# szpiech/garlic

Measured on AMD Instinct MI355X. Metric: LOD-windows/sec (SNPs x inds / winsize), higher is better.
Workload: dtype f64

## Files before the change

### garlic_amd/csrc/garlic_hip.hip

```cpp
#include "../../include/garlic_hip.h"
#include "lod_kernels.hpp"
#include "variant_kernels.hpp"
#include "ld_kernels.hpp"
#include "tgls_ring_kernel.hpp"
#include "wlod_strip_kernel.hpp"
#include "wlod_small_kernel.hpp"
#include "coverage_kernel.hpp"
#include "roh_segments_kernel.hpp"
#include "feed_kernel.hpp"
#include "wlod_feed_kernel.hpp"

#include <algorithm>
#include <chrono>
#include <functional>
#include <mutex>
#include <queue>
#include <cmath>
#include <cstdarg>
#include <cstdio>
#include <cstdlib>
#include <cstring>
#include <string>
#include <thread>
#include <tuple>
// ... 124 lines not shown
};

static int score_alloc(garlic_ctx *ctx, size_t bytes, void **out);
static int score_free(garlic_ctx *ctx, void *ptr);

template <class T> struct PoolBuf : NoCopy {
    T *p = nullptr;
    garlic_ctx *ctx = nullptr;
    ~PoolBuf() { release(); }
    int reserve(garlic_ctx *c, size_t n)
    {
        release();
        void *q = nullptr;
        const int rc = score_alloc(c, std::max<size_t>(n, 1) * sizeof(T), &q);
        if (rc) return rc;
        p = (T *)q;
        ctx = c;
        return GARLIC_OK;
    }
    void release()
    {
        if (p) (void)score_free(ctx, p);
        p = nullptr;
    }
};


struct garlic_panel {
    garlic_ctx *ctx = nullptr;
    int32_t nchr = 0;
    int32_t nind = 0;
    int64_t nloci = 0;
    int64_t nind_pad = 0;
    int64_t nwordrows = 0;
    std::vector<int32_t> chr_nloci;
    std::vector<int64_t> chr_off;
    std::vector<int32_t> pos, cs, ce;
    std::vector<double> gpos, freq;
    bool have_map = false, have_freq = false, have_geno = false, have_gpos = false;
    DevBuf<uint32_t> d_packed;
    DevBuf<int32_t> d_pos, d_cs, d_ce;
    DevBuf<int64_t> d_chr_off;
    DevBuf<double> d_tab;
    bool tab_valid = false;
    double tab_error = 0;
    double tab_min = 0, tabgl_min = 0, glterms_min = 0;
    bool tab_all_finite = false;
    bool seg_valid = false;
    int32_t seg_max_gap = 0;
    std::vector<int64_t> boundaries;
    DevBuf<int32_t> d_blk_counts, d_blk_offsets, d_total;
    DevBuf<int64_t> d_boundaries;
    DevBuf<ChainItem> d_items;
    DevBuf<FeedItem> d_feed_items;
    DevBuf<FillItem> d_fill;
    DevBuf<int32_t> d_counter;
    DevBuf<ChrDev> d_chrs;
    DevBuf<int16_t> d_stage16;
    DevBuf<int64_t> d_row_counts;
    bool have_gl = false;
    std::vector<double> gl_values;
    std::unordered_map<uint64_t, int> gl_code;
    DevBuf<uint8_t> d_codes;
    DevBuf<double> d_tabgl;
    bool tabgl_valid = false;
    DevBuf<double> d_glterms;
    bool glterms_valid = false, glterms_scaled = false;
    int32_t glterms_M = 0;
    double glterms_mu = 0.0;

    int tabgl_ncodes = 0;
    bool gl_cont = false;
    DevBuf<double> d_glval;
    bool gl_vals_dropped = false;
    bool gl_cover_required = false;
    std::vector<uint8_t> gl_cover;
    DevBuf<double> d_freq;
    bool dfreq_valid = false;
    int gl_terms_by = 0;
    bool have_ld = false, wlod_use_gl = false, rld_valid = false;
    int32_t last_chain_kind = 0;
    int32_t last_feed_form = GARLIC_FEED_FROM_SCORES;
    int64_t last_feed_doubles = 0;
    int32_t ld_winsize = 0;
    DevBuf<double> d_rld, d_decay, d_stage64;
    DevBuf<uint64_t> d_phase;
    uint64_t geno_epoch = 0;
    CovBits cov_pending{nullptr, nullptr, 0.0};
    bool cov_written = false;
    bool have_phase = false;
    struct {
        DevBuf<uint64_t> sub, m, h, o;
        DevBuf<int32_t> loc, pair, loc_planes;
        DevBuf<double> hf, fwd, bwd, ld;
        DevBuf<LdSumChr> sum_chrs;
        DevBuf<LdPairChr> pair_chrs;
        uint64_t planes_key = 0;
        bool planes_valid = false;
        bool fuse_request = false, fused_done = false;
        void release()
        {
            sub.release(); m.release(); h.release(); o.release(); loc.release(); pair.release(); loc_planes.release();
            hf.release(); fwd.release(); bwd.release(); ld.release(); sum_chrs.release(); pair_chrs.release();
            planes_valid = false;
        }
    } lds;
// ... 916 lines not shown
    if (wlod_shape_ok && use_gl && (rc = ensure_gl_terms(p, true, c.M, c.mu))) return rc;
    f.wlod_gl = wlod_shape_ok && use_gl && p->glterms_valid && p->glterms_scaled;
    f.wlod_tuned = (wlod_shape_ok && !use_gl) || f.wlod_gl;
    if (f.wlod_tuned && !f.wlod_gl && sizeof(double) * (size_t)(W + TILE) * 4 + 16 > 150 * 1024) f.wlod_tuned = false;
    if (f.wlod_tuned && !f.wlod_gl && (rc = ensure_score_rows(p, c.error, c.M, c.mu, W))) return rc;
    if (!f.wlod_tuned && (rc = ensure_rld(p))) return rc;
    const bool wlod_stream = f.wlod_tuned && wlod_small && !f.cov_bits && !getenv("GARLIC_WLOD_SMALL_TILES");
    if (f.cov_bits && !f.wlod_tuned) return GARLIC_INTERNAL_NO_BITS;
    if (wlod_stream && (rc = ensure_rld(p))) return rc;
    if (use_gl && p->gl_cont && !f.wlod_tuned && (rc = ensure_gl_terms(p))) return rc;
    if (!f.wlod_tuned) {
        f.family = Family::wlod_generic;
        return GARLIC_OK;
    }
    f.writes_bits = true;
    f.no_prefetch = getenv("GARLIC_WLOD_NO_PF") != nullptr;
    const size_t wlod_rows = f.wlod_gl ? 0 : sizeof(double) * (size_t)(W + TILE) * 4;
    const size_t wlod_patch = sizeof(double) * (size_t)WAVE * WT_PITCH;
    const bool wlod_use_patch = wlod_rows + 16 + wlod_patch <= 160 * 1024 / 8 && !getenv("GARLIC_WLOD_NO_PATCH");
    const bool wlod_gl_ring = f.wlod_gl && !wlod_small && (c.ind_begin & (WAVE - 1)) == 0 && !getenv("GARLIC_WLOD_GL_NO_RING");
    const bool ring_patch = !getenv("GARLIC_WLOD_GL_NO_PATCH");
    const int strip_waves = (W + 15 - 16 * WS_WAVES <= 16 || getenv("GARLIC_WLOD_STRIP_NARROW_ONLY")) ? WS_WAVES : WS_WAVES_WIDE;
    const bool wlod_gl_strip = wlod_gl_ring && W + 15 - 16 * strip_waves <= 16 && !getenv("GARLIC_WLOD_GL_NO_STRIP");
    f.strip_waves = strip_waves;
    f.use_patch = wlod_gl_ring ? ring_patch : wlod_use_patch;
    f.tile_lds = wlod_gl_ring ? WLOD_GL_RING_OFF + (size_t)WLOD_WAVES * GARLIC_WLOD_GL_RING_ROWS * WAVE * 8
                              : wlod_rows + 16 + (wlod_use_patch ? wlod_patch : 0);
    f.strip_force_rerun = wlod_gl_strip && getenv("GARLIC_WLOD_STRIP_FORCE_RERUN") != nullptr;
    f.family = wlod_stream                            ? Family::wlod_stream
               : wlod_small                           ? Family::wlod_small_tiles
               : wlod_gl_strip                        ? Family::wlod_strip
               : wlod_gl_ring                         ? Family::wlod_glring
               : f.wlod_gl                            ? Family::wlod_tile_gl
               : !getenv("GARLIC_WLOD_ONE_BLOCK")     ? Family::wlod_tile2
                                                      : Family::wlod_tile;
    return GARLIC_OK;
}

void finish_form(const garlic_panel *p, const LodCall &c, const Layout &L, const double *d_out, LodForm &f)
{
    f.aligned16 = (c.pitch_align % 2 == 0) && ((reinterpret_cast<uintptr_t>(d_out) & 15) == 0);
    if (f.family == Family::wlod_stream && !f.aligned16) f.family = Family::wlod_small_tiles;
    f.strip_three = f.family == Family::wlod_strip && f.strip_waves != WS_WAVES_WIDE && f.aligned16 && !f.cov_bits &&
                    !getenv("GARLIC_WLOD_STRIP_TWO_PER_CU");
    for (int k = 0; f.strip_three && k < p->nchr; k++) f.strip_three = L.pitch[k] * 8 < ((int64_t)1 << 32);
}

using Plan = garlic_panel::Plan;

struct LodWork {
    std::vector<Run> runs;
    std::vector<FillItem> fill;
    std::vector<ChainItem> items;
    std::vector<FeedItem> feed_items;
    std::vector<ChrDev> chrs;
    std::vector<uint8_t> valid;
    std::vector<int2> tiles, segs;
    std::vector<WlodStrip> strips;
    std::vector<int32_t> feed_blocks;
};

int plan_lod(garlic_panel *p, const LodCall &c, const LodForm &form, const Layout &L, const garlic_panel::PlanKey &key, LodWork &w, Plan &plan)
{
    plan = Plan{false, key};
    const int nblk = (c.ind_count + WAVE - 1) / WAVE;
    int rc;
    p->plan.valid = false;
    plan_runs(p, c.W, w.runs, w.fill, plan.n_valid);
    const std::vector<int> order = longest_first(w.runs);
    w.items.reserve(w.runs.size() * nblk);
    for (size_t i = 0; i < order.size(); i++) {
        const Run &r = w.runs[order[i]];
        for (int k = 0; k < nblk; k++)
            if (!c.blocks || (*c.blocks)[(size_t)k]) w.items.push_back(ChainItem{r.chr, r.a, r.b, k * WAVE});
    }
    if (form.family == Family::feed) {
        std::vector<int32_t> col0(w.runs.size());
        for (size_t i = 0; i < w.runs.size(); i++) {
            const int32_t s = (w.runs[i].a + c.thin_step - 1) / c.thin_step;
            col0[i] = (int64_t)s * c.thin_step <= w.runs[i].b ? s : -1;
        }
        build_feed_items(w.runs, order, c.blocks, nblk, col0, w.feed_items);
        plan.n_feed_items = w.feed_items.size();
    }
    w.chrs.resize(p->nchr);
    for (int k = 0; k < p->nchr; k++)
        w.chrs[k] = ChrDev{p->chr_off[k], L.base[k], L.pitch[k], p->chr_nloci[k],
                           (c.pitch_align >= 2 && 64 * L.pitch[k] * 8 + 512 < ((int64_t)1 << 32)) ? 1 : 0};
    plan.n_items = w.items.size();
    plan.n_fill = w.fill.size();
    plan.n_runs = (int64_t)w.runs.size();
    if (!p->d_counter.p) {
        if ((rc = p->d_counter.reserve(8))) return rc;
        HIP_TRY(hipMemsetAsync(p->d_counter.p, 0, 8 * sizeof(int32_t), p->ctx->stream));
    }
    if (form.wlod_tuned || form.family == Family::wlod_feed) {
        w.valid.assign((size_t)p->nloci, 0);
        for (const Run &r : w.runs)
            memset(w.valid.data() + p->chr_off[r.chr] + r.a, 1, (size_t)(r.b - r.a + 1));
    }
    if (form.family == Family::wlod_feed) {
        for (int k = 0; k < p->nchr; k++) {
            const int32_t cols = (int32_t)(((int64_t)p->chr_nloci[k] + c.thin_step - 1) / c.thin_step);
            for (int32_t c0 = 0; c0 < cols; c0 += WFD_COLS) w.tiles.push_back(make_int2(k, c0));
        }
        plan.n_tiles = (int32_t)w.tiles.size();
        for (int k = 0; k < nblk; k++)
            if (!c.blocks || (*c.blocks)[(size_t)k]) w.feed_blocks.push_back(k);
        plan.n_feed_blocks = (int32_t)w.feed_blocks.size();
    }
    if (form.wlod_tuned) {
        for (int k = 0; k < p->nchr; k++)
            for (int s0 = 0; s0 < p->chr_nloci[k]; s0 += TILE) w.tiles.push_back(make_int2(k, s0));
        plan.n_tiles = (int32_t)w.tiles.size();
        for (int k = 0; k < p->nchr; k++)
            for (int s0 = 0; s0 < p->chr_nloci[k]; s0 += WSM_T) w.segs.push_back(make_int2(k, s0));
        plan.n_segs = (int32_t)w.segs.size();
    }
    if (form.family == Family::wlod_strip) {
        int64_t total_groups = 0;
        for (int k = 0; k < p->nchr; k++) total_groups += (p->chr_nloci[k] + WLOD_R - 1) / WLOD_R;
        const int64_t pairs = (nblk + 1) / 2;
        int64_t per = total_groups * pairs / 8192;
        per = std::min<int64_t>(256, std::max<int64_t>(64, per)) & ~(int64_t)1;
        if (const char *e = getenv("GARLIC_WLOD_STRIP_GROUPS")) per = std::max<int64_t>(1, atol(e));
        for (int k = 0; k < p->nchr; k++) {
            const int ng = (p->chr_nloci[k] + WLOD_R - 1) / WLOD_R;
            for (int g0 = 0; g0 < ng; g0 += (int)per)
                w.strips.push_back(WlodStrip{k, g0 * WLOD_R, std::min<int>((int)per, ng - g0), 0});
        }
        plan.n_strips = (int32_t)w.strips.size();
    }
    return GARLIC_OK;
}

int score_buffer(garlic_panel *p, const LodCall &c, const Layout &L, double **d_out)
{
    *d_out = c.out;
    if (c.where != GARLIC_HOST) return GARLIC_OK;
    int rc;
    if (p->d_out.cap < (size_t)L.total && c.mode == MODE_LOD && c.thin_step == 0 && !p->placing &&
// ... 75 lines not shown
int launch_wlod(garlic_panel *p, const LodCall &c, const LodForm &form, const Plan &plan, double *d_out)
{
    hipStream_t s = p->ctx->stream;
    const int nblk = (c.ind_count + WAVE - 1) / WAVE;
    const int per_wg = form.family == Family::wlod_tile2 ? WLOD2_BLOCKS : WLOD_WAVES;
    const int nquad = (nblk + per_wg - 1) / per_wg;
    const bool gl_ring = form.family == Family::wlod_glring || form.family == Family::wlod_strip;
    const int64_t score_rows = GOFF + p->nloci + GPAD_BACK;
    WlodArgs a{p->d_valid.p, p->d_chrs.p, p->d_tiles.p, p->nwordrows, p->nchr, c.ind_begin, c.ind_count, c.W, nquad,
               (uint32_t)((int64_t)plan.n_tiles * nquad), (form.use_patch ? 1 : 0) | (form.no_prefetch ? 2 : 0),
               score_rows, gl_ring ? 1 : 0, p->cov_pending, nullptr, nullptr};
    const uint32_t *a_packed = p->d_packed.p;
    const double *a_wtab = form.wlod_gl ? p->d_glterms.p : p->d_wtab.p, *a_skew = p->d_skew.p + SKEW_FRONT;
    const dim3 wl_block(WLOD_WAVES * WAVE);
    if (form.family == Family::wlod_stream) {
        a.tiles = p->d_segs.p;
        a.nquad = (nblk + WLOD2_BLOCKS - 1) / WLOD2_BLOCKS;
        a.n_work = (uint32_t)((int64_t)plan.n_segs * a.nquad);
        a.use_patch = 1;
        const void *fn = form.wlod_gl ? wlod_stream_small_gl_fn(c.W) : wlod_stream_small_fn(c.W);
        const size_t lds = wlod_small_lds_bytes(c.W);
        if (lds > 48 * 1024) HIP_TRY(hipFuncSetAttribute(fn, hipFuncAttributeMaxDynamicSharedMemorySize, (int)lds));
        const double *a_rld = p->d_rld.p;
        void *kargs[] = {(void *)&a_packed, (void *)&a_wtab, (void *)&a_rld, (void *)&d_out, (void *)&a};
        HIP_TRY(hipLaunchKernel(fn, dim3((a.n_work + 7u) / 8u * 8u), wl_block, kargs, lds, s));
        return GARLIC_OK;
    }
    if (form.family == Family::wlod_strip) {
        const int n_pairs = (nblk + 1) / 2;
        WlodStripArgs sa{p->d_valid.p, p->d_chrs.p, p->d_strips.p, p->d_glterms.p, a_skew, d_out,
                         score_rows, c.ind_begin, c.ind_count, c.W, form.strip_waves, n_pairs,
                         form.use_patch ? 1 : 0, (uint32_t)((int64_t)plan.n_strips * n_pairs), p->d_counter.p + 3, p->cov_pending};
        HIP_TRY(hipMemsetAsync(p->d_counter.p + 3, 0, sizeof(int32_t), s));
        const void *fn = form.strip_three ? (const void *)wlod_strip_gl3_kernel
                         : form.strip_waves == WS_WAVES_WIDE ? (form.aligned16 ? (const void *)wlod_strip_gl_kernel<true, WS_WAVES_WIDE>
                                                  : (const void *)wlod_strip_gl_kernel<false, WS_WAVES_WIDE>)
                                : (form.aligned16 ? (const void *)wlod_strip_gl_kernel<true, WS_WAVES>
                                                  : (const void *)wlod_strip_gl_kernel<false, WS_WAVES>);
        const uint32_t strip_lds = form.strip_three ? WF_LDS_BYTES : WS_LDS_BYTES;
        HIP_TRY(hipFuncSetAttribute(fn, hipFuncAttributeMaxDynamicSharedMemorySize, (int)strip_lds));
        void *kargs[] = {(void *)&sa};
        HIP_TRY(hipLaunchKernel(fn, dim3((sa.n_work + 7u) / 8u * 8u), dim3((form.strip_waves + 1) * WAVE), kargs, strip_lds, s));
        if (form.strip_force_rerun) HIP_TRY(hipMemsetAsync(p->d_counter.p + 3, 1, sizeof(int32_t), s));
        a.run_if = p->d_counter.p + 3;
        a.rerun_count = p->d_counter.p + 4;
    }
    const void *fn = wlod_tile_fn(form.family, form.wlod_gl, form.aligned16);
    if (form.tile_lds > 48 * 1024) HIP_TRY(hipFuncSetAttribute(fn, hipFuncAttributeMaxDynamicSharedMemorySize, (int)form.tile_lds));
    void *kargs[] = {(void *)&a_packed, (void *)&a_wtab, (void *)&a_skew, (void *)&d_out, (void *)&a};
    HIP_TRY(hipLaunchKernel(fn, dim3((a.n_work + 7u) / 8u * 8u), wl_block, kargs, form.tile_lds, s));
    return GARLIC_OK;
}

int launch_chain(garlic_panel *p, const LodCall &c, const LodForm &form, Plan &plan, const LodWork *fresh, int workers, double *d_out)
{
    garlic_ctx *ctx = p->ctx;
    ItemTrace trace;
    if (form.family == Family::feed && plan.n_feed_items) {
        FeedArgs f{p->d_packed.p, p->d_tab.p, p->d_feed_items.p, p->d_chrs.p, d_out, nullptr, p->nwordrows, c.ind_begin, c.ind_count, c.W,
                   (int32_t)plan.n_feed_items, c.thin_step, form.feed_asm ? 1 : 0, p->d_counter.p, nullptr};
        f.trace = trace.begin(8, plan.n_feed_items, "\n", ctx->stream);
        int grid = (int)std::min<size_t>(plan.n_feed_items, (size_t)ctx->n_cu * std::max(1, plan.feed_per_cu)), rc;
        if (fresh && (rc = feed_grid(ctx, fresh->feed_items, &grid, &plan.feed_per_cu))) return rc;
        void *kargs[] = {(void *)&f};
        HIP_TRY(hipLaunchKernel((const void *)lod_feed_kernel, dim3((unsigned)grid), dim3(FEED_G * WAVE), kargs, 0, ctx->stream));
    } else {
        ChainArgs a{p->d_packed.p, p->d_tab.p, p->d_items.p,     p->d_chrs.p,          d_out, p->nind_pad, p->nwordrows,
                    c.ind_begin,   c.ind_count, c.W,             (int32_t)plan.n_items, p->d_counter.p, nullptr};
        a.trace = trace.begin(4, plan.n_items, " 0\n", ctx->stream);
        if (form.aligned16)
            hipLaunchKernelGGL((lod_chain_kernel<true>), dim3((unsigned)workers), dim3(CHAIN_THREADS), 0, ctx->stream, a);
        else
            hipLaunchKernelGGL((lod_chain_kernel<false>), dim3((unsigned)workers), dim3(CHAIN_THREADS), 0, ctx->stream, a);
    }
    trace.write(ctx->stream);
    return GARLIC_OK;
}

int launch_tgls(garlic_panel *p, const LodCall &c, const LodForm &form, const Plan &plan, int workers, double *d_out)
{
    hipStream_t s = p->ctx->stream;
    const int64_t rows = GOFF + p->nloci + GPAD_BACK;
    if (form.cov_bits && !form.writes_bits) return GARLIC_INTERNAL_NO_BITS;
    if (form.family == Family::tgls_ring) {
        TglsArgs t{p->d_glterms.p, rows, p->d_items.p, p->d_chrs.p, d_out,
                   c.ind_begin, c.ind_count, c.W, (int32_t)plan.n_items, p->d_counter.p, p->cov_pending};
        if (form.cov_bits) p->cov_written = true;
        hipLaunchKernelGGL(lod_chain_ring_kernel, dim3((unsigned)workers), dim3(TG_THREADS), 0, s, t);
        return GARLIC_OK;
    }
    const VariantArgs a = variant_args(p, c, form, d_out);
    if (form.family == Family::tgls_terms)
        hipLaunchKernelGGL(lod_chain_terms_kernel, dim3((unsigned)plan.n_items), dim3(2 * WAVE), 0, s, a, (int)plan.n_items, rows, p->d_glterms.p);
    else
        hipLaunchKernelGGL(lod_chain_gl_kernel, dim3((unsigned)((plan.n_items + GL_WAVES - 1) / GL_WAVES)), dim3(GL_WAVES * WAVE), 0, s, a,
                           (int)plan.n_items);
    return GARLIC_OK;
}

int launch_generic_wlod(garlic_panel *p, const LodCall &c, const LodForm &form, const Plan &plan, double *d_out)
{
    const int ring = c.W + TILE;
    const size_t lds = sizeof(double) * ((size_t)ring * WAVE + ((c.W + 1) & ~1) + (size_t)WAVE * TPITCH);
    if (lds > 160 * 1024)
        return fail(GARLIC_ERR_INVALID, "wLOD with winsize %d: this build supports 2..240 and 16..4096", c.W);
    HIP_TRY(hipFuncSetAttribute(reinterpret_cast<const void *>(wlod_kernel), hipFuncAttributeMaxDynamicSharedMemorySize, (int)lds));
    hipLaunchKernelGGL(wlod_kernel, dim3((unsigned)plan.n_items), dim3(WAVE), lds, p->ctx->stream, variant_args(p, c, form, d_out), ring);
    return GARLIC_OK;
}

int launch_wlod_feed(garlic_panel *p, const LodCall &c, const LodForm &form, const Plan &plan, double *d_out)
{
    const int nquad = (plan.n_feed_blocks + WFD_WAVES - 1) / WFD_WAVES;
    WlodFeedArgs a{p->d_packed.p, form.wlod_gl ? p->d_glterms.p : p->d_wtab.p, p->d_skew.p + SKEW_FRONT, p->d_valid.p, p->d_chrs.p,
                   p->d_tiles.p, p->d_feed_blocks.p, d_out, p->nwordrows, GOFF + p->nloci + GPAD_BACK, c.ind_count, c.W, c.thin_step,
                   plan.n_feed_blocks, nquad, (uint32_t)((int64_t)plan.n_tiles * nquad)};
    if (!a.n_work) return GARLIC_OK;
    if (form.wlod_gl) hipLaunchKernelGGL(wlod_feed_kernel<true>, dim3(a.n_work), dim3(WFD_WAVES * WAVE), 0, p->ctx->stream, a);
    else hipLaunchKernelGGL(wlod_feed_kernel<false>, dim3(a.n_work), dim3(WFD_WAVES * WAVE), 0, p->ctx->stream, a);
    return GARLIC_OK;
}

int enqueue_lod(garlic_panel *p, const LodCall &c, const LodForm &form, const Layout &L, Plan &plan, const LodWork *fresh,
                double *d_out, Family family)
{
    garlic_ctx *ctx = p->ctx;
    hipStream_t s = ctx->stream;
    int rc = GARLIC_OK;
    HIP_TRY(hipEventRecord(ctx->ev_begin, s));
    if (fresh && ((rc = p->d_chrs.put(fresh->chrs, s)) || (rc = p->d_items.put(fresh->items, s)) || (rc = p->d_fill.put(fresh->fill, s)) ||
                  (rc = p->d_feed_items.put(fresh->feed_items, s)) || (rc = p->d_valid.put(fresh->valid, s)) ||
                  (rc = p->d_tiles.put(fresh->tiles, s)) || (rc = p->d_segs.put(fresh->segs, s)) || (rc = p->d_strips.put(fresh->strips, s)) ||
                  (rc = p->d_feed_blocks.put(fresh->feed_blocks, s))))
        return rc;
    if (family == Family::feed) {
        hipLaunchKernelGGL(fill_value_kernel, dim3(1024), dim3(256), 0, s, d_out, L.total, MISSING_D);
    } else if (plan.n_fill && !form.wlod_tuned && family != Family::wlod_feed && !form.cov_bits) {
        dim3 grid((unsigned)plan.n_fill, (unsigned)((c.ind_count + FILL_ROWS - 1) / FILL_ROWS));
        hipLaunchKernelGGL(fill_missing_kernel, grid, dim3(256), 0, s, p->d_fill.p, p->d_chrs.p, c.ind_count, d_out);
    }
    if (plan.n_items && (fresh || c.mode != MODE_LOD)) HIP_TRY(hipMemsetAsync(p->d_counter.p, 0, 2 * sizeof(int32_t), s));
    p->stats_slot = (int)(ctx->n_calls % garlic_ctx::HIST);
    HIP_TRY(hist_mark(ctx, false));
    int workers = ctx->n_cu;
    if (const char *e = getenv("GARLIC_WORKERS")) workers = std::max(1, atoi(e));
    workers = std::min<int>(workers, (int)plan.n_items);
    if (form.wlod_tuned || plan.n_items || family == Family::wlod_feed)
        switch (family) {
        case Family::chain:
        case Family::feed: rc = launch_chain(p, c, form, plan, fresh, workers, d_out); break;
        case Family::exact:
            hipLaunchKernelGGL(lod_chain_exact_kernel, dim3((unsigned)plan.n_items), dim3(WAVE), 0, s, variant_args(p, c, form, d_out),
                               (int)plan.n_items);
            break;
        case Family::tgls_ring:
        case Family::tgls_terms:
        case Family::tgls_lookup: rc = launch_tgls(p, c, form, plan, workers, d_out); break;
        case Family::wlod_generic: rc = launch_generic_wlod(p, c, form, plan, d_out); break;
        case Family::wlod_feed: rc = launch_wlod_feed(p, c, form, plan, d_out); break;
        default: rc = launch_wlod(p, c, form, plan, d_out);
        }
    if (rc) return rc;
    HIP_TRY(hist_mark(ctx, true));
    HIP_TRY(hipGetLastError());
    return GARLIC_OK;
}

int launch_lod(garlic_panel *p, Mode mode, int32_t W, double error, int32_t max_gap, int32_t M, double mu,
               int32_t ind_begin, int32_t ind_count, int32_t pitch_align, double *out, int32_t where,
               int32_t thin_step = 0, const std::vector<uint8_t> *blocks = nullptr)
{
    garlic_ctx *ctx = p->ctx;
    int rc;
    if ((rc = set_device(ctx))) return rc;
    const LodCall c{mode, W, max_gap, M, ind_begin, ind_count, where == GARLIC_HOST ? std::max(pitch_align, 32) : pitch_align,
                    thin_step, where, pitch_align, error, mu, out, blocks};
    LodForm form;
    if ((rc = check_lod_args(p, c)) || (rc = decide_form(p, c, form))) return rc;
    const Layout Lhost = make_layout(p, pitch_align, ind_count), L = make_layout(p, c.pitch_align, ind_count, thin_step);
    for (int k = 0; k < p->nchr; k++)
        if (3 * L.pitch[k] * 8 + 512 >= (int64_t)1 << 32)
            return fail(GARLIC_ERR_INVALID, "chromosome %d too long for 32-bit row offsets", k);
    double *d_out = nullptr;
    if ((rc = score_buffer(p, c, L, &d_out))) return rc;
    finish_form(p, c, L, d_out, form);

    garlic_panel::PlanKey key{(int)mode, W, max_gap, ind_begin, ind_count, c.pitch_align, thin_step, 0, form.wlod_tuned,
                form.family == Family::wlod_strip, thin_step > 0};
    if (blocks) {
// ... 1936 lines not shown
```

### garlic_amd/csrc/lod_kernels.hpp

```cpp
#pragma once
#include <hip/hip_runtime.h>
#include <stdint.h>

#include "chain_loop_gfx950.inc"

namespace garlic {

constexpr int WAVE = 64;
constexpr int TILE = 32;
constexpr int TPITCH = 34;
constexpr int GOFF = 32;
constexpr int GPAD_CHAIN = 32 * GARLIC_CHAIN_NSLOT + 48 * GARLIC_CHAIN_CHROWS + 64;
constexpr int GPAD_BACK = GPAD_CHAIN > 4160 ? GPAD_CHAIN : 4160;
constexpr double MISSING_D = -9999.0;

struct ChrDev {
    int64_t loc_base;
    int64_t out_base;
    int64_t out_pitch;
    int32_t nloci;
    int32_t fast;
};

struct ChainItem {
// ... 137 lines not shown
seg_scan_kernel(const int32_t *block_counts, int nblocks, int32_t *block_offsets, int32_t *total)
{
    int carry = 0;
    for (int base = 0; base < nblocks; base += WAVE) {
        int i = base + threadIdx.x;
        int v = (i < nblocks) ? block_counts[i] : 0;
        int inc = wave_inclusive_scan(v);
        if (i < nblocks) block_offsets[i] = carry + inc - v;
        carry += __shfl(inc, WAVE - 1, WAVE);
    }
    if (threadIdx.x == 0) *total = carry;
}

__global__ void __launch_bounds__(SEG_BLOCK)
seg_compact_kernel(const int32_t *pos, const int64_t *chr_off, const int32_t *cs,
                   const int32_t *ce, int nchr, int64_t nloci, int32_t max_gap,
                   const int32_t *block_offsets, int64_t *boundaries)
{
    __shared__ int wsum[SEG_BLOCK / WAVE];
    __shared__ int running;
    if (threadIdx.x == 0) running = block_offsets[blockIdx.x];
    int64_t base = (int64_t)blockIdx.x * SEG_BLOCK * SEG_ITEMS;
    __syncthreads();
    for (int k = 0; k < SEG_ITEMS; k++) {
        int64_t G = base + (int64_t)k * SEG_BLOCK + threadIdx.x;
        int f = boundary_flag(pos, chr_off, cs, ce, nchr, nloci, max_gap, G);
        int inc = wave_inclusive_scan(f);
        if ((threadIdx.x & 63) == 63) wsum[threadIdx.x >> 6] = inc;
        __syncthreads();
        int woff = 0;
        for (int w = 0; w < (int)(threadIdx.x >> 6); w++) woff += wsum[w];
        int start = running;
        if (f) boundaries[start + woff + inc - 1] = G;
        __syncthreads();
        if (threadIdx.x == SEG_BLOCK - 1) running = start + woff + inc;
        __syncthreads();
    }
}

constexpr int FILL_ROWS = 16;
__global__ void __launch_bounds__(256)
fill_missing_kernel(const FillItem *items, const ChrDev *chrs, int32_t nind, double *out)
{
    FillItem it = items[blockIdx.x];
    ChrDev c = chrs[it.chr];
    int wave = threadIdx.x >> 6, lane = threadIdx.x & 63;
    int row0 = blockIdx.y * FILL_ROWS;
    for (int r = row0 + wave; r < row0 + FILL_ROWS && r < nind; r += 4) {
        double *row = out + c.out_base + (int64_t)r * c.out_pitch;
        for (int l = it.lo + lane; l < it.hi; l += WAVE) row[l] = MISSING_D;
    }
}

struct ChainArgs {
    const uint32_t *packed;
    const double *tab;
    const ChainItem *items;
    const ChrDev *chrs;
    double *out;
    int64_t nind_pad;
    int64_t nwordrows;
    int32_t ind_begin;
    int32_t ind_count;
    int32_t winsize;
    int32_t n_items;
    int32_t *next_item;
    int64_t *trace;
};

constexpr uint32_t SLOT_BYTES = 3072;
constexpr uint32_t SL_LW1 = 0, SL_LW2 = 256, SL_TW1 = 512, SL_TW2 = 768;
constexpr uint32_t SL_LTAB = 1024, SL_TTAB = 2048;
constexpr uint32_t LDS_ITEM = 3072;
constexpr uint32_t LDS_TILE = GARLIC_CHAIN_LDS_TILE0;
constexpr uint32_t LDS_BYTES = GARLIC_CHAIN_LDS_TOTAL;
constexpr int CHAIN_THREADS = 256;

struct Streams {
    int64_t lead_w, trail_w;
    const double *lead_tab, *trail_tab;
    int sh_lead, sh_trail;
};

__device__ __forceinline__ void advance(Streams &st)
{
    st.lead_w += 2; st.trail_w += 2;
    st.lead_tab += 4 * TILE; st.trail_tab += 4 * TILE;
}

__device__ __forceinline__ void fill_regs(unsigned char *smem, const Streams &st,
                                          const uint32_t *gcol, int lane)
{
    const uint32_t l1 = gcol[(st.lead_w + 1) * WAVE], l2 = gcol[(st.lead_w + 2) * WAVE];
    const uint32_t t1 = gcol[(st.trail_w + 1) * WAVE], t2 = gcol[(st.trail_w + 2) * WAVE];
    const double2 tl = reinterpret_cast<const double2 *>(st.lead_tab)[lane];
    const double2 tt = reinterpret_cast<const double2 *>(st.trail_tab)[lane];
    *reinterpret_cast<uint32_t *>(smem + SL_LW1 + lane * 4) = l1;
    *reinterpret_cast<uint32_t *>(smem + SL_LW2 + lane * 4) = l2;
    *reinterpret_cast<uint32_t *>(smem + SL_TW1 + lane * 4) = t1;
    *reinterpret_cast<uint32_t *>(smem + SL_TW2 + lane * 4) = t2;
    *reinterpret_cast<double2 *>(smem + SL_LTAB + lane * 16) = tl;
    *reinterpret_cast<double2 *>(smem + SL_TTAB + lane * 16) = tt;
}

struct TileBits {
    uint32_t lead_lo, lead_hi, trail_lo, trail_hi;
};

template <int SLOT>
__device__ __forceinline__ TileBits tile_consume(const unsigned char *smem, uint32_t &lc,
                                                 uint32_t &tc, const Streams &st, int lane)
{
    const unsigned char *slot = smem + SLOT * SLOT_BYTES;
    const uint32_t l1 = *reinterpret_cast<const uint32_t *>(slot + SL_LW1 + lane * 4);
    const uint32_t l2 = *reinterpret_cast<const uint32_t *>(slot + SL_LW2 + lane * 4);
    const uint32_t t1 = *reinterpret_cast<const uint32_t *>(slot + SL_TW1 + lane * 4);
    const uint32_t t2 = *reinterpret_cast<const uint32_t *>(slot + SL_TW2 + lane * 4);
    TileBits tb;
    tb.lead_lo = __builtin_amdgcn_alignbit(l1, lc, st.sh_lead);
    tb.lead_hi = __builtin_amdgcn_alignbit(l2, l1, st.sh_lead);
    tb.trail_lo = __builtin_amdgcn_alignbit(t1, tc, st.sh_trail);
    tb.trail_hi = __builtin_amdgcn_alignbit(t2, t1, st.sh_trail);
    lc = l2;
    tc = t2;
    return tb;
}
// ... 6 lines not shown
    const unsigned char *slot = smem + SLOT * SLOT_BYTES;
    const uint32_t tile_lane = (uint32_t)lane * (TPITCH * 8);
#pragma unroll
    for (int j = 0; j < TILE; j++) {
        const uint32_t lw = (j < 16) ? tb.lead_lo : tb.lead_hi;
        const uint32_t tw = (j < 16) ? tb.trail_lo : tb.trail_hi;
        const uint32_t g1 = (lw >> (2 * (j & 15))) & 3u;
        const uint32_t g0 = (tw >> (2 * (j & 15))) & 3u;
        double t_in = *reinterpret_cast<const double *>(slot + SL_LTAB + j * 32 + g1 * 8);
        double t_out = *reinterpret_cast<const double *>(slot + SL_TTAB + j * 32 + g0 * 8);
        if (EDGE) {
            const int s = s0 + j;
            if (!(s > a && s <= b)) t_out = 0.0;
            if (!(s >= a && s <= b)) t_in = 0.0;
        }
        acc = (acc - t_out) + t_in;
        *reinterpret_cast<double *>(tile + tile_lane + j * 8) = acc;
    }
}

template <bool EDGE, bool ALIGNED16>
__device__ __forceinline__ void tile_store(const unsigned char *tile, int s0, int a, int b, int lane,
                                           int rows_valid, double *out_tile, int64_t pitch)
{
    const int rsub = lane >> 4, csub = lane & 15;
#pragma unroll
    for (int q = 0; q < WAVE / 4; q++) {
        const int qe = (4 * q < rows_valid) ? q : 0;
        const int re = min(rsub, rows_valid - 1 - 4 * qe);
        const double2 v = *reinterpret_cast<const double2 *>(
            tile + (uint32_t)(4 * qe + re) * (TPITCH * 8) + csub * 16);
        char *base = reinterpret_cast<char *>(out_tile + (int64_t)(4 * qe) * pitch);
        const uint32_t off = (uint32_t)re * (uint32_t)(pitch * 8) + (uint32_t)csub * 16u;
        double *dst = reinterpret_cast<double *>(base + off);
        if (EDGE) {
            const int s = s0 + 2 * csub;
            if (s >= a && s <= b) dst[0] = v.x;
            if (s + 1 >= a && s + 1 <= b) dst[1] = v.y;
        } else if (!ALIGNED16) {
            dst[0] = v.x;
            dst[1] = v.y;
        } else {
            *reinterpret_cast<double2 *>(dst) = v;
        }
    }
}

__global__ void __launch_bounds__(256) fill_value_kernel(double *dst, int64_t n, double value)
{
    for (int64_t i = (int64_t)blockIdx.x * blockDim.x + threadIdx.x; i < n; i += (int64_t)gridDim.x * blockDim.x)
        dst[i] = value;
}

template <bool ALIGNED16>
__global__ void __launch_bounds__(CHAIN_THREADS)
lod_chain_kernel(ChainArgs p)
{
    __shared__ __attribute__((aligned(16))) unsigned char smem[LDS_BYTES];
    unsigned char *tile = smem + LDS_TILE;
    const int lane = threadIdx.x & (WAVE - 1);
    const int wave = __builtin_amdgcn_readfirstlane(threadIdx.x >> 6);
    for (;;) {
    if (threadIdx.x == 0)
        *reinterpret_cast<int *>(smem + LDS_ITEM) = atomicAdd(p.next_item, 1);
    __syncthreads();
    const int item_idx =
        __builtin_amdgcn_readfirstlane(*reinterpret_cast<const int *>(smem + LDS_ITEM));
    __syncthreads();
    if (item_idx >= p.n_items) {
        if (threadIdx.x == 0) {
            __threadfence();
            if (atomicAdd(p.next_item + 1, 1) == (int)gridDim.x - 1) {
                p.next_item[0] = 0;
                p.next_item[1] = 0;
            }
        }
        return;
    }
    if (p.trace && threadIdx.x == 0) {
        p.trace[4 * item_idx + 0] = blockIdx.x;
        p.trace[4 * item_idx + 1] = wall_clock64();
    }
    const ChainItem it = p.items[item_idx];
    const ChrDev c = p.chrs[it.chr];
    const int W = p.winsize;
    const int a = it.a, b = it.b;
    const int rows_valid = min(WAVE, p.ind_count - it.ind0);
    const int64_t col0 = (int64_t)p.ind_begin + it.ind0;
    const uint32_t *gcol = p.packed + packed_index(0, col0 + lane, p.nwordrows);
    const int64_t Gbase = c.loc_base + GOFF;

    double acc = 0.0;
    if (wave == 0) {
        int l = a;
        const int lend = a + W - 1;
        while (l < lend) {
            const int64_t G = Gbase + l;
            const int sh = 2 * (int)(G & 15);
            const uint32_t *wp = gcol + (G >> 4) * WAVE;
            uint32_t wd[5];
#pragma unroll
            for (int q = 0; q < 5; q++) wd[q] = wp[q * WAVE];
            uint32_t al[4];
#pragma unroll
            for (int q = 0; q < 4; q++) al[q] = __builtin_amdgcn_alignbit(wd[q + 1], wd[q], sh);
            const int n = min(64, lend - l);
            double t[64];
#pragma unroll
            for (int q = 0; q < 64; q++) {
                const uint32_t g = (al[q >> 4] >> (2 * (q & 15))) & 3u;
                t[q] = p.tab[(G + min(q, n - 1)) * 4 + ((q < n) ? g : 3u)];
            }
#pragma unroll
            for (int q = 0; q < 64; q++) acc += (q < n) ? t[q] : 0.0;
            l += n;
        }
    }

    int s0 = a & ~(TILE - 1);
    Streams st;
    {
        const int64_t Glead = Gbase + s0 + W - 1;
        const int64_t Gtrail = Gbase + s0 - 1;
        st.sh_lead = 2 * (int)(Glead & 15);
        st.sh_trail = 2 * (int)(Gtrail & 15);
        st.lead_w = Glead >> 4;
        st.trail_w = Gtrail >> 4;
        st.lead_tab = p.tab + Glead * 4;
        st.trail_tab = p.tab + Gtrail * 4;
    }
    double *const out_row = p.out + c.out_base + (int64_t)it.ind0 * c.out_pitch;
    double *out_tile = out_row + s0;
    const int64_t pitch = c.out_pitch;

    for (int phase = 0; phase < 2; phase++) {
        const int last = (phase == 0) ? s0 : b;
        while (s0 <= last && s0 <= b) {
            if (wave == 0) {
                uint32_t lc = gcol[st.lead_w * WAVE];
                uint32_t tc = gcol[st.trail_w * WAVE];
                fill_regs(smem, st, gcol, lane);
                const TileBits tb = tile_consume<0>(smem, lc, tc, st, lane);
                tile_steps<true, 0>(smem, tile, acc, tb, s0, a, b, lane);
                tile_store<true, ALIGNED16>(tile, s0, a, b, lane, rows_valid, out_tile, pitch);
            }
            advance(st);
            s0 += TILE;
            out_tile += TILE;
        }
        if (phase == 1 || !ALIGNED16 || !c.fast || (col0 & 63) != 0) continue;
        if (st.lead_w - st.trail_w > GARLIC_CHAIN_MAX_DW) continue;

        int ntiles = (b + 1 - s0) / TILE;
        if (ntiles >= 2) {
            uint32_t lc = gcol[st.lead_w * WAVE];
            uint32_t tc = gcol[st.trail_w * WAVE];
            const int64_t chunk0 = st.trail_w / GARLIC_CHAIN_CHROWS;
            const int64_t chunkI = (st.lead_w + 2 * GARLIC_CHAIN_NSLOT) / GARLIC_CHAIN_CHROWS + 1;
            const uint32_t *pchunk =
                p.packed + packed_index(GARLIC_CHAIN_CHROWS * chunk0, col0, p.nwordrows);
            const uint32_t wmask = GARLIC_CHAIN_WROWS - 1;
            if (p.trace && threadIdx.x == 0) p.trace[4 * item_idx + 2] = wall_clock64();
            const uint32_t a_nchunk0 = (uint32_t)(chunkI - chunk0 + 1) * (GARLIC_CHAIN_CHROWS / 4);
            const uint32_t a_roff0 = (uint32_t)((GARLIC_CHAIN_CHROWS * chunk0) & wmask) * 256u;
            const uint32_t a_laddr0 = (uint32_t)(st.lead_w & wmask) * 256u;
            const uint32_t a_taddr0 = (uint32_t)(st.trail_w & wmask) * 256u;
            if (wave == 0) {
                uint32_t tin[4], tout[4];
#pragma unroll
                for (int q = 0; q < 4; q++) {
                    const uint32_t bb = 4u * (uint32_t)lane + (uint32_t)q;
                    const uint32_t sp = (bb & 3u) | (((bb >> 2) & 3u) << 8) | (((bb >> 4) & 3u) << 16) | (((bb >> 6) & 3u) << 24);
                    tin[q] = sp << 4;
                    tout[q] = sp << 6;
                }
                *reinterpret_cast<uint4 *>(smem + GARLIC_CHAIN_SPREAD_IN + lane * 16) = make_uint4(tin[0], tin[1], tin[2], tin[3]);
                *reinterpret_cast<uint4 *>(smem + GARLIC_CHAIN_SPREAD_OUT + lane * 16) = make_uint4(tout[0], tout[1], tout[2], tout[3]);
            }
            {
                asm volatile(GARLIC_CHAIN_LOOP_ASM
                             : [acc] "+v"(acc)
                             : [wave] "s"(wave), [lane] "v"(lane), [lc] "v"(lc), [tc] "v"(tc),
                               [pchunk] "s"(pchunk), [nchunk0] "s"(a_nchunk0), [roff0] "s"(a_roff0),
                               [laddr0] "s"(a_laddr0), [taddr0] "s"(a_taddr0),
                               [pltab] "s"(st.lead_tab), [pttab] "s"(st.trail_tab), [out] "s"(out_tile),
                               [ntiles] "s"(ntiles), [shl] "s"(st.sh_lead), [sht] "s"(st.sh_trail),
                               [pitch8] "s"((uint32_t)(pitch * 8)), [rows] "s"(rows_valid)
                             : GARLIC_CHAIN_LOOP_CLOBBERS);
            }
            st.lead_w += 2 * ntiles;
            st.trail_w += 2 * ntiles;
            st.lead_tab += (int64_t)(4 * TILE) * ntiles;
            st.trail_tab += (int64_t)(4 * TILE) * ntiles;
            s0 += ntiles * TILE;
            out_tile += (int64_t)ntiles * TILE;
            __syncthreads();
        }
    }
    if (p.trace && threadIdx.x == 0) p.trace[4 * item_idx + 3] = wall_clock64();
    }
}

}
```

Baseline: 7.293 billion.

## Split chain kernel into prep pass plus prefetched per-item start records

Moves each chain item's serial warm-up (initial window sum and first partial tile) into a separate chain_prep_kernel that runs one item per wave across many blocks, and also folds the missing-value fill into that launch. Per-item scalar setup (offsets, shifts, chunk addresses) is now computed on the host into 128-byte ChainStart records. The main persistent kernel has a spare wave fetch the next item index and record into LDS while the current item runs, so the atomic grab and setup latency overlap with work. The cost is an extra kernel launch, a device buffer for per-lane prep state, more host planning work, and a tail loop that now runs after the asm fast path rather than before it.

Measured after the change: 7.276 billion, median of 2. No clear change (-0.2%).

```diff
diff --git a/garlic_amd/csrc/garlic_hip.hip b/garlic_amd/csrc/garlic_hip.hip
--- a/garlic_amd/csrc/garlic_hip.hip
+++ b/garlic_amd/csrc/garlic_hip.hip
@@ -200,6 +200,8 @@
     DevBuf<int32_t> d_blk_counts, d_blk_offsets, d_total;
     DevBuf<int64_t> d_boundaries;
     DevBuf<ChainItem> d_items;
+    DevBuf<ChainStart> d_starts;
+    DevBuf<PrepRec> d_prep;
     DevBuf<FeedItem> d_feed_items;
     DevBuf<FillItem> d_fill;
     DevBuf<int32_t> d_counter;
@@ -1222,6 +1224,7 @@
     std::vector<Run> runs;
     std::vector<FillItem> fill;
     std::vector<ChainItem> items;
+    std::vector<ChainStart> starts;
     std::vector<FeedItem> feed_items;
     std::vector<ChrDev> chrs;
     std::vector<uint8_t> valid;
@@ -1229,6 +1232,46 @@
     std::vector<WlodStrip> strips;
     std::vector<int32_t> feed_blocks;
 };
+
+void chain_starts(const garlic_panel *p, const LodCall &c, const std::vector<ChrDev> &chrs, const std::vector<ChainItem> &items,
+                  std::vector<ChainStart> &starts)
+{
+    starts.resize(items.size());
+    for (size_t i = 0; i < items.size(); i++) {
+        const ChainItem &it = items[i];
+        const ChrDev &ch = chrs[(size_t)it.chr];
+        ChainStart &r = starts[i];
+        memset(&r, 0, sizeof(r));
+        const int64_t Gbase = ch.loc_base + GOFF;
+        const int64_t col0 = (int64_t)c.ind_begin + it.ind0;
+        r.a = it.a;
+        r.b = it.b;
+        r.s1 = (it.a & ~(TILE - 1)) + TILE;
+        r.rows_valid = std::min<int32_t>(WAVE, c.ind_count - it.ind0);
+        r.col0 = (int32_t)col0;
+        r.pitch = ch.out_pitch;
+        r.out_off = ch.out_base + (int64_t)it.ind0 * ch.out_pitch + r.s1;
+        const int64_t Glead = Gbase + r.s1 + c.W - 1, Gtrail = Gbase + r.s1 - 1;
+        r.sh_lead = 2 * (int32_t)(Glead & 15);
+        r.sh_trail = 2 * (int32_t)(Gtrail & 15);
+        r.lead_w = (int32_t)(Glead >> 4);
+        r.trail_w = (int32_t)(Gtrail >> 4);
+        r.lead_tab_off = Glead * 4;
+        r.trail_tab_off = Gtrail * 4;
+        const bool fast = ch.fast && (col0 & 63) == 0 && r.lead_w - r.trail_w <= GARLIC_CHAIN_MAX_DW;
+        const int32_t ntiles = r.s1 <= it.b ? (it.b + 1 - r.s1) / TILE : 0;
+        r.ntiles = (fast && ntiles >= 2) ? ntiles : 0;
+        const int64_t chunk0 = r.trail_w / GARLIC_CHAIN_CHROWS;
+        const int64_t chunkI = ((int64_t)r.lead_w + 2 * GARLIC_CHAIN_NSLOT) / GARLIC_CHAIN_CHROWS + 1;
+        const uint32_t wmask = GARLIC_CHAIN_WROWS - 1;
+        r.pchunk_off = packed_index(GARLIC_CHAIN_CHROWS * chunk0, col0, p->nwordrows);
+        r.nchunk0 = (uint32_t)(chunkI - chunk0 + 1) * (GARLIC_CHAIN_CHROWS / 4);
+        r.roff0 = (uint32_t)((GARLIC_CHAIN_CHROWS * chunk0) & wmask) * 256u;
+        r.laddr0 = (uint32_t)r.lead_w & wmask;
+        r.laddr0 *= 256u;
+        r.taddr0 = ((uint32_t)r.trail_w & wmask) * 256u;
+    }
+}
 
 int plan_lod(garlic_panel *p, const LodCall &c, const LodForm &form, const Layout &L, const garlic_panel::PlanKey &key, LodWork &w, Plan &plan)
 {
@@ -1257,6 +1300,7 @@
     for (int k = 0; k < p->nchr; k++)
         w.chrs[k] = ChrDev{p->chr_off[k], L.base[k], L.pitch[k], p->chr_nloci[k],
                            (c.pitch_align >= 2 && 64 * L.pitch[k] * 8 + 512 < ((int64_t)1 << 32)) ? 1 : 0};
+    if (c.mode == MODE_LOD && c.thin_step == 0) chain_starts(p, c, w.chrs, w.items, w.starts);
     plan.n_items = w.items.size();
     plan.n_fill = w.fill.size();
     plan.n_runs = (int64_t)w.runs.size();
@@ -1438,6 +1482,13 @@
     return GARLIC_OK;
 }
 
+ChainArgs chain_args(const garlic_panel *p, const LodCall &c, const Plan &plan, double *d_out)
+{
+    return ChainArgs{p->d_packed.p, p->d_tab.p, p->d_items.p, p->d_chrs.p, p->d_starts.p, p->d_prep.p, p->d_fill.p, d_out,
+                     p->nind_pad, p->nwordrows, c.ind_begin, c.ind_count, c.W, (int32_t)plan.n_items, (int32_t)plan.n_fill,
+                     p->d_counter.p, nullptr};
+}
+
 int launch_chain(garlic_panel *p, const LodCall &c, const LodForm &form, Plan &plan, const LodWork *fresh, int workers, double *d_out)
 {
     garlic_ctx *ctx = p->ctx;
@@ -1451,8 +1502,7 @@
         void *kargs[] = {(void *)&f};
         HIP_TRY(hipLaunchKernel((const void *)lod_feed_kernel, dim3((unsigned)grid), dim3(FEED_G * WAVE), kargs, 0, ctx->stream));
     } else {
-        ChainArgs a{p->d_packed.p, p->d_tab.p, p->d_items.p,     p->d_chrs.p,          d_out, p->nind_pad, p->nwordrows,
-                    c.ind_begin,   c.ind_count, c.W,             (int32_t)plan.n_items, p->d_counter.p, nullptr};
+        ChainArgs a = chain_args(p, c, plan, d_out);
         a.trace = trace.begin(4, plan.n_items, " 0\n", ctx->stream);
         if (form.aligned16)
             hipLaunchKernelGGL((lod_chain_kernel<true>), dim3((unsigned)workers), dim3(CHAIN_THREADS), 0, ctx->stream, a);
@@ -1515,12 +1565,17 @@
     int rc = GARLIC_OK;
     HIP_TRY(hipEventRecord(ctx->ev_begin, s));
     if (fresh && ((rc = p->d_chrs.put(fresh->chrs, s)) || (rc = p->d_items.put(fresh->items, s)) || (rc = p->d_fill.put(fresh->fill, s)) ||
+                  (rc = p->d_starts.put(fresh->starts, s)) || (rc = p->d_prep.reserve(fresh->starts.size() * WAVE)) ||
                   (rc = p->d_feed_items.put(fresh->feed_items, s)) || (rc = p->d_valid.put(fresh->valid, s)) ||
                   (rc = p->d_tiles.put(fresh->tiles, s)) || (rc = p->d_segs.put(fresh->segs, s)) || (rc = p->d_strips.put(fresh->strips, s)) ||
                   (rc = p->d_feed_blocks.put(fresh->feed_blocks, s))))
         return rc;
     if (family == Family::feed) {
         hipLaunchKernelGGL(fill_value_kernel, dim3(1024), dim3(256), 0, s, d_out, L.total, MISSING_D);
+    } else if (family == Family::chain) {
+        const ChainArgs a = chain_args(p, c, plan, d_out);
+        const size_t grid = (plan.n_items + 3) / 4 + plan.n_fill * (size_t)((c.ind_count + FILL_ROWS - 1) / FILL_ROWS);
+        if (grid) hipLaunchKernelGGL(chain_prep_kernel, dim3((unsigned)grid), dim3(256), 0, s, a);
     } else if (plan.n_fill && !form.wlod_tuned && family != Family::wlod_feed && !form.cov_bits) {
         dim3 grid((unsigned)plan.n_fill, (unsigned)((c.ind_count + FILL_ROWS - 1) / FILL_ROWS));
         hipLaunchKernelGGL(fill_missing_kernel, grid, dim3(256), 0, s, p->d_fill.p, p->d_chrs.p, c.ind_count, d_out);
diff --git a/garlic_amd/csrc/lod_kernels.hpp b/garlic_amd/csrc/lod_kernels.hpp
--- a/garlic_amd/csrc/lod_kernels.hpp
+++ b/garlic_amd/csrc/lod_kernels.hpp
@@ -213,11 +213,37 @@
     }
 }
 
+struct alignas(128) ChainStart {
+    int64_t out_off;
+    int64_t lead_tab_off;
+    int64_t trail_tab_off;
+    int64_t pchunk_off;
+    int64_t pitch;
+    int32_t a, b;
+    int32_t s1;
+    int32_t rows_valid;
+    int32_t ntiles;
+    int32_t col0;
+    int32_t lead_w, trail_w;
+    int32_t sh_lead, sh_trail;
+    uint32_t nchunk0, roff0, laddr0, taddr0;
+};
+constexpr int CHAIN_START_WORDS = 24;
+static_assert(sizeof(ChainStart) == 128 && offsetof(ChainStart, taddr0) == 4 * (CHAIN_START_WORDS - 1), "ChainStart layout");
+
+struct alignas(16) PrepRec {
+    double acc;
+    uint32_t lc, tc;
+};
+
 struct ChainArgs {
     const uint32_t *packed;
     const double *tab;
     const ChainItem *items;
     const ChrDev *chrs;
+    const ChainStart *starts;
+    PrepRec *prep;
+    const FillItem *fill;
     double *out;
     int64_t nind_pad;
     int64_t nwordrows;
@@ -225,6 +251,7 @@
     int32_t ind_count;
     int32_t winsize;
     int32_t n_items;
+    int32_t n_fill;
     int32_t *next_item;
     int64_t *trace;
 };
@@ -233,6 +260,7 @@
 constexpr uint32_t SL_LW1 = 0, SL_LW2 = 256, SL_TW1 = 512, SL_TW2 = 768;
 constexpr uint32_t SL_LTAB = 1024, SL_TTAB = 2048;
 constexpr uint32_t LDS_ITEM = 3072;
+constexpr uint32_t LDS_START = 3200;
 constexpr uint32_t LDS_TILE = GARLIC_CHAIN_LDS_TILE0;
 constexpr uint32_t LDS_BYTES = GARLIC_CHAIN_LDS_TOTAL;
 constexpr int CHAIN_THREADS = 256;
@@ -345,35 +373,31 @@
         dst[i] = value;
 }
 
-template <bool ALIGNED16>
-__global__ void __launch_bounds__(CHAIN_THREADS)
-lod_chain_kernel(ChainArgs p)
-{
-    __shared__ __attribute__((aligned(16))) unsigned char smem[LDS_BYTES];
-    unsigned char *tile = smem + LDS_TILE;
+constexpr uint32_t PREP_WAVE_LDS = SLOT_BYTES + WAVE * TPITCH * 8;
+__global__ void __launch_bounds__(256)
+chain_prep_kernel(ChainArgs p)
+{
+    __shared__ __attribute__((aligned(16))) unsigned char smem_all[4 * PREP_WAVE_LDS];
     const int lane = threadIdx.x & (WAVE - 1);
     const int wave = __builtin_amdgcn_readfirstlane(threadIdx.x >> 6);
-    for (;;) {
-    if (threadIdx.x == 0)
-        *reinterpret_cast<int *>(smem + LDS_ITEM) = atomicAdd(p.next_item, 1);
-    __syncthreads();
-    const int item_idx =
-        __builtin_amdgcn_readfirstlane(*reinterpret_cast<const int *>(smem + LDS_ITEM));
-    __syncthreads();
-    if (item_idx >= p.n_items) {
-        if (threadIdx.x == 0) {
-            __threadfence();
-            if (atomicAdd(p.next_item + 1, 1) == (int)gridDim.x - 1) {
-                p.next_item[0] = 0;
-                p.next_item[1] = 0;
-            }
+    const int n_head = (p.n_items + 3) >> 2;
+    if ((int)blockIdx.x >= n_head) {
+        const int row_groups = (p.ind_count + FILL_ROWS - 1) / FILL_ROWS;
+        const int f = ((int)blockIdx.x - n_head) / row_groups;
+        if (f >= p.n_fill) return;
+        const FillItem it = p.fill[f];
+        const ChrDev c = p.chrs[it.chr];
+        const int row0 = (((int)blockIdx.x - n_head) - f * row_groups) * FILL_ROWS;
+        for (int r = row0 + wave; r < row0 + FILL_ROWS && r < p.ind_count; r += 4) {
+            double *row = p.out + c.out_base + (int64_t)r * c.out_pitch;
+            for (int l = it.lo + lane; l < it.hi; l += WAVE) row[l] = MISSING_D;
         }
         return;
     }
-    if (p.trace && threadIdx.x == 0) {
-        p.trace[4 * item_idx + 0] = blockIdx.x;
-        p.trace[4 * item_idx + 1] = wall_clock64();
-    }
+    const int item_idx = (int)blockIdx.x * 4 + wave;
+    if (item_idx >= p.n_items) return;
+    unsigned char *smem = smem_all + wave * PREP_WAVE_LDS;
+    unsigned char *tile = smem + SLOT_BYTES;
     const ChainItem it = p.items[item_idx];
     const ChrDev c = p.chrs[it.chr];
     const int W = p.winsize;
@@ -384,33 +408,31 @@
     const int64_t Gbase = c.loc_base + GOFF;
 
     double acc = 0.0;
-    if (wave == 0) {
-        int l = a;
-        const int lend = a + W - 1;
-        while (l < lend) {
-            const int64_t G = Gbase + l;
-            const int sh = 2 * (int)(G & 15);
-            const uint32_t *wp = gcol + (G >> 4) * WAVE;
-            uint32_t wd[5];
-#pragma unroll
-            for (int q = 0; q < 5; q++) wd[q] = wp[q * WAVE];
-            uint32_t al[4];
-#pragma unroll
-            for (int q = 0; q < 4; q++) al[q] = __builtin_amdgcn_alignbit(wd[q + 1], wd[q], sh);
-            const int n = min(64, lend - l);
-            double t[64];
-#pragma unroll
-            for (int q = 0; q < 64; q++) {
-                const uint32_t g = (al[q >> 4] >> (2 * (q & 15))) & 3u;
-                t[q] = p.tab[(G + min(q, n - 1)) * 4 + ((q < n) ? g : 3u)];
-            }
-#pragma unroll
-            for (int q = 0; q < 64; q++) acc += (q < n) ? t[q] : 0.0;
-            l += n;
-        }
-    }
-
-    int s0 = a & ~(TILE - 1);
+    int l = a;
+    const int lend = a + W - 1;
+    while (l < lend) {
+        const int64_t G = Gbase + l;
+        const int sh = 2 * (int)(G & 15);
+        const uint32_t *wp = gcol + (G >> 4) * WAVE;
+        uint32_t wd[5];
+#pragma unroll
+        for (int q = 0; q < 5; q++) wd[q] = wp[q * WAVE];
+        uint32_t al[4];
+#pragma unroll
+        for (int q = 0; q < 4; q++) al[q] = __builtin_amdgcn_alignbit(wd[q + 1], wd[q], sh);
+        const int n = min(64, lend - l);
+        double t[64];
+#pragma unroll
+        for (int q = 0; q < 64; q++) {
+            const uint32_t g = (al[q >> 4] >> (2 * (q & 15))) & 3u;
+            t[q] = p.tab[(G + min(q, n - 1)) * 4 + ((q < n) ? g : 3u)];
+        }
+#pragma unroll
+        for (int q = 0; q < 64; q++) acc += (q < n) ? t[q] : 0.0;
+        l += n;
+    }
+
+    const int s0 = a & ~(TILE - 1);
     Streams st;
     {
         const int64_t Glead = Gbase + s0 + W - 1;
@@ -422,73 +444,131 @@
         st.lead_tab = p.tab + Glead * 4;
         st.trail_tab = p.tab + Gtrail * 4;
     }
-    double *const out_row = p.out + c.out_base + (int64_t)it.ind0 * c.out_pitch;
-    double *out_tile = out_row + s0;
-    const int64_t pitch = c.out_pitch;
-
-    for (int phase = 0; phase < 2; phase++) {
-        const int last = (phase == 0) ? s0 : b;
-        while (s0 <= last && s0 <= b) {
-            if (wave == 0) {
-                uint32_t lc = gcol[st.lead_w * WAVE];
-                uint32_t tc = gcol[st.trail_w * WAVE];
-                fill_regs(smem, st, gcol, lane);
-                const TileBits tb = tile_consume<0>(smem, lc, tc, st, lane);
-                tile_steps<true, 0>(smem, tile, acc, tb, s0, a, b, lane);
-                tile_store<true, ALIGNED16>(tile, s0, a, b, lane, rows_valid, out_tile, pitch);
+    double *out_tile = p.out + c.out_base + (int64_t)it.ind0 * c.out_pitch + s0;
+    uint32_t lc = gcol[st.lead_w * WAVE];
+    uint32_t tc = gcol[st.trail_w * WAVE];
+    fill_regs(smem, st, gcol, lane);
+    const TileBits tb = tile_consume<0>(smem, lc, tc, st, lane);
+    tile_steps<true, 0>(smem, tile, acc, tb, s0, a, b, lane);
+    tile_store<true, false>(tile, s0, a, b, lane, rows_valid, out_tile, c.out_pitch);
+    PrepRec r;
+    r.acc = acc;
+    r.lc = lc;
+    r.tc = tc;
+    p.prep[(int64_t)item_idx * WAVE + lane] = r;
+}
+
+__device__ __forceinline__ void chain_grab(const ChainArgs &p, unsigned char *smem, int lane)
+{
+    int idx = 0;
+    if (lane == 0) idx = atomicAdd(p.next_item, 1);
+    idx = __builtin_amdgcn_readfirstlane(idx);
+    uint32_t v = 0;
+    if (idx < p.n_items && lane < CHAIN_START_WORDS) v = reinterpret_cast<const uint32_t *>(p.starts + idx)[lane];
+    if (lane == 0) *reinterpret_cast<int *>(smem + LDS_ITEM) = idx;
+    if (lane < CHAIN_START_WORDS) *reinterpret_cast<uint32_t *>(smem + LDS_START + lane * 4) = v;
+}
+
+template <bool ALIGNED16>
+__global__ void __launch_bounds__(CHAIN_THREADS)
+lod_chain_kernel(ChainArgs p)
+{
+    __shared__ __attribute__((aligned(16))) unsigned char smem[LDS_BYTES];
+    unsigned char *tile = smem + LDS_TILE;
+    const int lane = threadIdx.x & (WAVE - 1);
+    const int wave = __builtin_amdgcn_readfirstlane(threadIdx.x >> 6);
+    if (wave == 1) chain_grab(p, smem, lane);
+    for (;;) {
+    __syncthreads();
+    const int item_idx =
+        __builtin_amdgcn_readfirstlane(*reinterpret_cast<const int *>(smem + LDS_ITEM));
+    const uint32_t start_word = *reinterpret_cast<const uint32_t *>(smem + LDS_START + (lane & 31) * 4);
+    __syncthreads();
+    if (item_idx >= p.n_items) {
+        if (threadIdx.x == 0) {
+            __threadfence();
+            if (atomicAdd(p.next_item + 1, 1) == (int)gridDim.x - 1) {
+                p.next_item[0] = 0;
+                p.next_item[1] = 0;
             }
+        }
+        return;
+    }
+    if (p.trace && threadIdx.x == 0) {
+        p.trace[4 * item_idx + 0] = blockIdx.x;
+        p.trace[4 * item_idx + 1] = wall_clock64();
+    }
+    ChainStart c;
+    {
+        uint32_t w[CHAIN_START_WORDS];
+#pragma unroll
+        for (int q = 0; q < CHAIN_START_WORDS; q++) w[q] = (uint32_t)__builtin_amdgcn_readlane((int)start_word, q);
+        __builtin_memcpy(&c, w, sizeof(w));
+    }
+    const PrepRec pr = p.prep[(int64_t)item_idx * WAVE + lane];
+    double acc = pr.acc;
+    const int a = c.a, b = c.b;
+    const int rows_valid = c.rows_valid;
+    int s0 = c.s1;
+    Streams st;
+    st.sh_lead = c.sh_lead;
+    st.sh_trail = c.sh_trail;
+    st.lead_w = c.lead_w;
+    st.trail_w = c.trail_w;
+    st.lead_tab = p.tab + c.lead_tab_off;
+    st.trail_tab = p.tab + c.trail_tab_off;
+    double *out_tile = p.out + c.out_off;
+    const int64_t pitch = c.pitch;
+
+    if (ALIGNED16 && c.ntiles >= 2) {
+        const int ntiles = c.ntiles;
+        const uint32_t *pchunk = p.packed + c.pchunk_off;
+        if (p.trace && threadIdx.x == 0) p.trace[4 * item_idx + 2] = wall_clock64();
+        if (wave == 0) {
+            uint32_t tin[4], tout[4];
+#pragma unroll
+            for (int q = 0; q < 4; q++) {
+                const uint32_t bb = 4u * (uint32_t)lane + (uint32_t)q;
+                const uint32_t sp = (bb & 3u) | (((bb >> 2) & 3u) << 8) | (((bb >> 4) & 3u) << 16) | (((bb >> 6) & 3u) << 24);
+                tin[q] = sp << 4;
+                tout[q] = sp << 6;
+            }
+            *reinterpret_cast<uint4 *>(smem + GARLIC_CHAIN_SPREAD_IN + lane * 16) = make_uint4(tin[0], tin[1], tin[2], tin[3]);
+            *reinterpret_cast<uint4 *>(smem + GARLIC_CHAIN_SPREAD_OUT + lane * 16) = make_uint4(tout[0], tout[1], tout[2], tout[3]);
+        }
+        {
+            asm volatile(GARLIC_CHAIN_LOOP_ASM
+                         : [acc] "+v"(acc)
+                         : [wave] "s"(wave), [lane] "v"(lane), [lc] "v"(pr.lc), [tc] "v"(pr.tc),
+                           [pchunk] "s"(pchunk), [nchunk0] "s"(c.nchunk0), [roff0] "s"(c.roff0),
+                           [laddr0] "s"(c.laddr0), [taddr0] "s"(c.taddr0),
+                           [pltab] "s"(st.lead_tab), [pttab] "s"(st.trail_tab), [out] "s"(out_tile),
+                           [ntiles] "s"(ntiles), [shl] "s"(st.sh_lead), [sht] "s"(st.sh_trail),
+                           [pitch8] "s"((uint32_t)(pitch * 8)), [rows] "s"(rows_valid)
+                         : GARLIC_CHAIN_LOOP_CLOBBERS);
+        }
+        st.lead_w += 2 * ntiles;
+        st.trail_w += 2 * ntiles;
+        st.lead_tab += (int64_t)(4 * TILE) * ntiles;
+        st.trail_tab += (int64_t)(4 * TILE) * ntiles;
+        s0 += ntiles * TILE;
+        out_tile += (int64_t)ntiles * TILE;
+        __syncthreads();
+    }
+    if (wave == 1) chain_grab(p, smem, lane);
+    if (wave == 0 && s0 <= b) {
+        const uint32_t *gcol = p.packed + packed_index(0, (int64_t)c.col0 + lane, p.nwordrows);
+        while (s0 <= b) {
+            uint32_t lc = gcol[st.lead_w * WAVE];
+            uint32_t tc = gcol[st.trail_w * WAVE];
+            fill_regs(smem, st, gcol, lane);
+            const TileBits tb = tile_consume<0>(smem, lc, tc, st, lane);
+            tile_steps<true, 0>(smem, tile, acc, tb, s0, a, b, lane);
+            tile_store<true, ALIGNED16>(tile, s0, a, b, lane, rows_valid, out_tile, pitch);
             advance(st);
             s0 += TILE;
             out_tile += TILE;
         }
-        if (phase == 1 || !ALIGNED16 || !c.fast || (col0 & 63) != 0) continue;
-        if (st.lead_w - st.trail_w > GARLIC_CHAIN_MAX_DW) continue;
-
-        int ntiles = (b + 1 - s0) / TILE;
-        if (ntiles >= 2) {
-            uint32_t lc = gcol[st.lead_w * WAVE];
-            uint32_t tc = gcol[st.trail_w * WAVE];
-            const int64_t chunk0 = st.trail_w / GARLIC_CHAIN_CHROWS;
-            const int64_t chunkI = (st.lead_w + 2 * GARLIC_CHAIN_NSLOT) / GARLIC_CHAIN_CHROWS + 1;
-            const uint32_t *pchunk =
-                p.packed + packed_index(GARLIC_CHAIN_CHROWS * chunk0, col0, p.nwordrows);
-            const uint32_t wmask = GARLIC_CHAIN_WROWS - 1;
-            if (p.trace && threadIdx.x == 0) p.trace[4 * item_idx + 2] = wall_clock64();
-            const uint32_t a_nchunk0 = (uint32_t)(chunkI - chunk0 + 1) * (GARLIC_CHAIN_CHROWS / 4);
-            const uint32_t a_roff0 = (uint32_t)((GARLIC_CHAIN_CHROWS * chunk0) & wmask) * 256u;
-            const uint32_t a_laddr0 = (uint32_t)(st.lead_w & wmask) * 256u;
-            const uint32_t a_taddr0 = (uint32_t)(st.trail_w & wmask) * 256u;
-            if (wave == 0) {
-                uint32_t tin[4], tout[4];
-#pragma unroll
-                for (int q = 0; q < 4; q++) {
-                    const uint32_t bb = 4u * (uint32_t)lane + (uint32_t)q;
-                    const uint32_t sp = (bb & 3u) | (((bb >> 2) & 3u) << 8) | (((bb >> 4) & 3u) << 16) | (((bb >> 6) & 3u) << 24);
-                    tin[q] = sp << 4;
-                    tout[q] = sp << 6;
-                }
-                *reinterpret_cast<uint4 *>(smem + GARLIC_CHAIN_SPREAD_IN + lane * 16) = make_uint4(tin[0], tin[1], tin[2], tin[3]);
-                *reinterpret_cast<uint4 *>(smem + GARLIC_CHAIN_SPREAD_OUT + lane * 16) = make_uint4(tout[0], tout[1], tout[2], tout[3]);
-            }
-            {
-                asm volatile(GARLIC_CHAIN_LOOP_ASM
-                             : [acc] "+v"(acc)
-                             : [wave] "s"(wave), [lane] "v"(lane), [lc] "v"(lc), [tc] "v"(tc),
-                               [pchunk] "s"(pchunk), [nchunk0] "s"(a_nchunk0), [roff0] "s"(a_roff0),
-                               [laddr0] "s"(a_laddr0), [taddr0] "s"(a_taddr0),
-                               [pltab] "s"(st.lead_tab), [pttab] "s"(st.trail_tab), [out] "s"(out_tile),
-                               [ntiles] "s"(ntiles), [shl] "s"(st.sh_lead), [sht] "s"(st.sh_trail),
-                               [pitch8] "s"((uint32_t)(pitch * 8)), [rows] "s"(rows_valid)
-                             : GARLIC_CHAIN_LOOP_CLOBBERS);
-            }
-            st.lead_w += 2 * ntiles;
-            st.trail_w += 2 * ntiles;
-            st.lead_tab += (int64_t)(4 * TILE) * ntiles;
-            st.trail_tab += (int64_t)(4 * TILE) * ntiles;
-            s0 += ntiles * TILE;
-            out_tile += (int64_t)ntiles * TILE;
-            __syncthreads();
-        }
     }
     if (p.trace && threadIdx.x == 0) p.trace[4 * item_idx + 3] = wall_clock64();
     }
```
